# traceopt-ai/traceml

Hardware: AMD Instinct MI355X
Metric: instrumentation overhead (% step time) (lower is better)
Workload: dtype bf16; 1 GPU; model=resnet50, global_batch=256, image_size=224, parallelism=dp1, protocol=plain

## Files before the change

traceml_amd/models/resnet.py:

```python

from __future__ import annotations

import torch
import torch.nn as nn


class Bottleneck(nn.Module):
    expansion = 4

    def __init__(self, in_ch: int, width: int, stride: int = 1):
        super().__init__()
        out_ch = width * self.expansion
        self.conv1 = nn.Conv2d(in_ch, width, 1, bias=False)
        self.bn1 = nn.BatchNorm2d(width)
        self.conv2 = nn.Conv2d(width, width, 3, stride=stride, padding=1, bias=False)
        self.bn2 = nn.BatchNorm2d(width)
        self.conv3 = nn.Conv2d(width, out_ch, 1, bias=False)
        self.bn3 = nn.BatchNorm2d(out_ch)
        self.relu = nn.ReLU(inplace=True)
        self.downsample = None
        if stride != 1 or in_ch != out_ch:
            self.downsample = nn.Sequential(
                nn.Conv2d(in_ch, out_ch, 1, stride=stride, bias=False),
                nn.BatchNorm2d(out_ch),
            )

    def forward(self, x):
        identity = x
        out = self.relu(self.bn1(self.conv1(x)))
        out = self.relu(self.bn2(self.conv2(out)))
        out = self.bn3(self.conv3(out))
        if self.downsample is not None:
            identity = self.downsample(x)
        return self.relu(out + identity)


class ResNet(nn.Module):
    def __init__(self, layers, num_classes: int = 1000):
        super().__init__()
        self.in_ch = 64
        self.conv1 = nn.Conv2d(3, 64, 7, stride=2, padding=3, bias=False)
        self.bn1 = nn.BatchNorm2d(64)
        self.relu = nn.ReLU(inplace=True)
        self.maxpool = nn.MaxPool2d(3, stride=2, padding=1)
        self.layer1 = self._make_layer(64, layers[0], stride=1)
        self.layer2 = self._make_layer(128, layers[1], stride=2)
        self.layer3 = self._make_layer(256, layers[2], stride=2)
        self.layer4 = self._make_layer(512, layers[3], stride=2)
        self.avgpool = nn.AdaptiveAvgPool2d(1)
        self.fc = nn.Linear(512 * Bottleneck.expansion, num_classes)
        for m in self.modules():
            if isinstance(m, nn.Conv2d):
                nn.init.kaiming_normal_(m.weight, mode="fan_out", nonlinearity="relu")
            elif isinstance(m, nn.BatchNorm2d):
                nn.init.ones_(m.weight)
                nn.init.zeros_(m.bias)

    def _make_layer(self, width, blocks, stride):
        layers = [Bottleneck(self.in_ch, width, stride)]
        self.in_ch = width * Bottleneck.expansion
        layers += [Bottleneck(self.in_ch, width) for _ in range(blocks - 1)]
        return nn.Sequential(*layers)

    def forward(self, x):
        x = self.maxpool(self.relu(self.bn1(self.conv1(x))))
        x = self.layer4(self.layer3(self.layer2(self.layer1(x))))
        x = torch.flatten(self.avgpool(x), 1)
        return self.fc(x)


def resnet50(num_classes: int = 1000) -> ResNet:
    return ResNet([3, 4, 6, 3], num_classes=num_classes)
```

traceml_amd/ops/build_ext.py:

```python

from __future__ import annotations

import os
import subprocess
import sys
import sysconfig

HERE = os.path.dirname(os.path.abspath(__file__))
SRC = os.path.join(HERE, "hip", "traceml_hip.hip")


def extension_filename() -> str:
    suffix = sysconfig.get_config_var("EXT_SUFFIX") or ".so"
    return os.path.join(HERE, f"_traceml_hip{suffix}")


def _pybind11_include() -> str:
    import pybind11

    return pybind11.get_include()


def build(verbose: bool = True) -> str:
    out = extension_filename()
    python_include = sysconfig.get_paths()["include"]
    cmd = [
        "hipcc",
        "--offload-arch=gfx950",
        "-O3",
        "-std=c++17",
        "-fPIC",
        "-shared",
        f"-I{python_include}",
        f"-I{_pybind11_include()}",
        SRC,
        "-o",
        out,
    ]
    if verbose:
        print("+", " ".join(cmd), flush=True)
    env = dict(os.environ)
    env.setdefault("PYTORCH_ROCM_ARCH", "gfx950")
    subprocess.run(cmd, check=True, env=env)
    return out


def build_if_needed(verbose: bool = True) -> str:
    out = extension_filename()
    if os.path.exists(out) and os.path.getmtime(out) >= os.path.getmtime(SRC):
        return out
    return build(verbose=verbose)


if __name__ == "__main__":
    build()
```

traceml_amd/ops/hip/traceml_hip.hip:

```cpp

#include <hip/hip_runtime.h>
#include <pybind11/pybind11.h>

#include <atomic>
#include <chrono>
#include <cstdint>
#include <cstring>
#include <mutex>
#include <stdexcept>
#include <string>
#include <thread>
#include <vector>

namespace py = pybind11;

#define HIP_CHECK(expr)                                                        \
  do {                                                                         \
    hipError_t _err = (expr);                                                  \
    if (_err != hipSuccess) {                                                  \
      throw std::runtime_error(std::string("HIP error at " #expr ": ") +       \
                               hipGetErrorString(_err));                       \
    }                                                                          \
  } while (0)

struct Slot {
  unsigned long long ticks;
  unsigned long long seq;
};
static_assert(sizeof(Slot) == 16, "slot must be 16 bytes");


__global__ __launch_bounds__(64, 1) void stamp_kernel(Slot* __restrict__ ring,
                                                      unsigned long long mask,
                                                      unsigned long long seq) {
  __shared__ Slot staged;
  if (threadIdx.x == 0) {
    staged.ticks = __builtin_amdgcn_s_memrealtime();
    staged.seq = seq;
    Slot* slot = ring + (seq & mask);
    slot->ticks = staged.ticks;
    __hip_atomic_store(&slot->seq, staged.seq, __ATOMIC_RELEASE,
                       __HIP_MEMORY_SCOPE_SYSTEM);
  }
}


namespace {

struct RingState {
  Slot* host_ptr = nullptr;
  Slot* dev_ptr = nullptr;
  unsigned long long capacity = 0;
  unsigned long long mask = 0;
  std::atomic<unsigned long long> next_seq{1};
  double ticks_per_sec = 0.0;
  int device = -1;
  bool initialized = false;
};

RingState g_ring;
std::mutex g_init_mutex;

struct EventPool {
  std::vector<hipEvent_t> events;
  std::vector<int> free_ids;
  std::mutex mutex;
};

EventPool g_events;

unsigned long long round_up_pow2(unsigned long long v) {
  unsigned long long p = 1;
  while (p < v) p <<= 1;
  return p;
}

double query_wall_clock_rate(int device) {
  int khz = 0;
  hipError_t err =
      hipDeviceGetAttribute(&khz, hipDeviceAttributeWallClockRate, device);
  if (err != hipSuccess || khz <= 0) return 0.0;
  return static_cast<double>(khz) * 1000.0;
}

}


static unsigned long long ring_mark(uintptr_t stream_handle) {
  RingState& r = g_ring;
  unsigned long long seq = r.next_seq.fetch_add(1, std::memory_order_relaxed);
  hipStream_t stream = reinterpret_cast<hipStream_t>(stream_handle);
  stamp_kernel<<<1, 64, 0, stream>>>(r.dev_ptr, r.mask, seq);
  return seq;
}

static bool ring_ready(unsigned long long seq) {
  const RingState& r = g_ring;
  const Slot* slot = r.host_ptr + (seq & r.mask);
  unsigned long long observed = __atomic_load_n(&slot->seq, __ATOMIC_ACQUIRE);
  return observed == seq;
}

static long long ring_ticks(unsigned long long seq) {
  const RingState& r = g_ring;
  const Slot* slot = r.host_ptr + (seq & r.mask);
  unsigned long long observed = __atomic_load_n(&slot->seq, __ATOMIC_ACQUIRE);
  if (observed != seq) return -1;
  return static_cast<long long>(slot->ticks);
}

static double ring_elapsed_ms(unsigned long long seq_start,
                              unsigned long long seq_end) {
  long long t0 = ring_ticks(seq_start);
  long long t1 = ring_ticks(seq_end);
  if (t0 < 0 || t1 < 0) return -1.0;
  double dticks = static_cast<double>(t1 - t0);
  return dticks * 1000.0 / g_ring.ticks_per_sec;
}

static double calibrate(uintptr_t stream_handle, double window_sec) {
  hipStream_t stream = reinterpret_cast<hipStream_t>(stream_handle);
  unsigned long long a = ring_mark(reinterpret_cast<uintptr_t>(stream));
  HIP_CHECK(hipStreamSynchronize(stream));
  auto cpu0 = std::chrono::steady_clock::now();
  long long ta = ring_ticks(a);
  std::this_thread::sleep_for(
      std::chrono::microseconds(static_cast<long long>(window_sec * 1e6)));
  unsigned long long b = ring_mark(reinterpret_cast<uintptr_t>(stream));
  HIP_CHECK(hipStreamSynchronize(stream));
  auto cpu1 = std::chrono::steady_clock::now();
  long long tb = ring_ticks(b);
  double sec =
      std::chrono::duration_cast<std::chrono::duration<double>>(cpu1 - cpu0)
          .count();
  if (ta < 0 || tb < 0 || sec <= 0.0) {
    throw std::runtime_error("traceml_hip: calibration stamps did not land");
  }
  double rate = static_cast<double>(tb - ta) / sec;
  g_ring.ticks_per_sec = rate;
  return rate;
}

static void init(int device, unsigned long long slots) {
  std::lock_guard<std::mutex> guard(g_init_mutex);
  if (g_ring.initialized) return;
  HIP_CHECK(hipSetDevice(device));
  unsigned long long capacity = round_up_pow2(slots < 1024 ? 1024 : slots);
  void* host = nullptr;
  HIP_CHECK(hipHostMalloc(&host, capacity * sizeof(Slot),
                          hipHostMallocMapped | hipHostMallocCoherent));
  std::memset(host, 0, capacity * sizeof(Slot));
  void* dev = nullptr;
  HIP_CHECK(hipHostGetDevicePointer(&dev, host, 0));
  g_ring.host_ptr = static_cast<Slot*>(host);
  g_ring.dev_ptr = static_cast<Slot*>(dev);
  g_ring.capacity = capacity;
  g_ring.mask = capacity - 1;
  g_ring.device = device;
  g_ring.ticks_per_sec = query_wall_clock_rate(device);
  g_ring.initialized = true;
  try {
    calibrate(0, 0.050);
  } catch (const std::exception&) {
    if (g_ring.ticks_per_sec <= 0.0) g_ring.ticks_per_sec = 1.0e8;
  }
}

static bool is_initialized() { return g_ring.initialized; }

static double ticks_per_second() { return g_ring.ticks_per_sec; }


static int event_acquire() {
  std::lock_guard<std::mutex> guard(g_events.mutex);
  if (!g_events.free_ids.empty()) {
    int id = g_events.free_ids.back();
    g_events.free_ids.pop_back();
    return id;
  }
  hipEvent_t event;
  HIP_CHECK(hipEventCreateWithFlags(&event, hipEventDefault));
  g_events.events.push_back(event);
  return static_cast<int>(g_events.events.size()) - 1;
}

static hipEvent_t event_for(int id) {
  if (id < 0 || id >= static_cast<int>(g_events.events.size())) {
    throw std::runtime_error("traceml_hip: bad event id");
  }
  return g_events.events[static_cast<size_t>(id)];
}

static void event_record(int id, uintptr_t stream_handle) {
  HIP_CHECK(hipEventRecord(event_for(id),
                           reinterpret_cast<hipStream_t>(stream_handle)));
}

static bool event_query(int id) {
  hipError_t err = hipEventQuery(event_for(id));
  if (err == hipSuccess) return true;
  if (err == hipErrorNotReady) return false;
  HIP_CHECK(err);
  return false;
}

static double event_elapsed_ms(int start_id, int end_id) {
  float ms = 0.0f;
  HIP_CHECK(hipEventElapsedTime(&ms, event_for(start_id), event_for(end_id)));
  return static_cast<double>(ms);
}

static void event_release(int id) {
  std::lock_guard<std::mutex> guard(g_events.mutex);
  event_for(id);
  g_events.free_ids.push_back(id);
}

static int event_pool_size() {
  std::lock_guard<std::mutex> guard(g_events.mutex);
  return static_cast<int>(g_events.events.size());
}


PYBIND11_MODULE(_traceml_hip, m) {
  m.doc() = "traceml_amd MI355X-native timing: s_memrealtime ring stamps + "
            "hipEvent pool (gfx950)";
  m.def("init", &init, py::arg("device"), py::arg("slots") = 65536);
  m.def("is_initialized", &is_initialized);
  m.def("ticks_per_second", &ticks_per_second);
  m.def("ring_mark", &ring_mark, py::arg("stream"));
  m.def("ring_ready", &ring_ready, py::arg("seq"));
  m.def("ring_ticks", &ring_ticks, py::arg("seq"));
  m.def("ring_elapsed_ms", &ring_elapsed_ms, py::arg("seq_start"),
        py::arg("seq_end"));
  m.def("calibrate", &calibrate, py::arg("stream") = 0,
        py::arg("window_sec") = 0.05);
  m.def("event_acquire", &event_acquire);
  m.def("event_record", &event_record, py::arg("event_id"), py::arg("stream"));
  m.def("event_query", &event_query, py::arg("event_id"));
  m.def("event_elapsed_ms", &event_elapsed_ms, py::arg("start_id"),
        py::arg("end_id"));
  m.def("event_release", &event_release, py::arg("event_id"));
  m.def("event_pool_size", &event_pool_size);
}
```

Before: 0.1093 percent.

## Add fused BatchNorm+residual+ReLU HIP kernels for ResNet bottlenecks

Adds custom HIP kernels that fuse training-mode BatchNorm statistics, affine apply, residual add and ReLU for NHWC bf16 tensors, with matching backward kernels. ResNet blocks now route through bn_act, which falls back to the module path when hooks are present or shapes are unsupported. The aim is to cut memory traffic and kernel launches in the model step. This changes the step time that is the denominator of the overhead metric, and it also interacts with instrumentation, because hooked modules bypass the fused path.

```diff
diff --git a/profiles/fused_bn_bytes.py b/profiles/fused_bn_bytes.py
--- /dev/null
+++ b/profiles/fused_bn_bytes.py
@@ -0,0 +1,81 @@
+#!/usr/bin/env python3
+
+import csv
+import sys
+
+BATCH = 256
+ROOF_TBS = 6.29
+
+
+def plan_grid(rows, channels):
+    r = 256 // (channels // 8)
+    per_block = -(-rows // 1024)
+    per_block = -(-per_block // r) * r
+    per_block = max(per_block, 8 * r, 64)
+    return -(-rows // per_block)
+
+
+def sites():
+    out = [(BATCH * 112 * 112, 64, False)]
+    hw, in_planes = 56, 64
+    for width, blocks, stride in ((64, 3, 1), (128, 4, 2), (256, 6, 2),
+                                  (512, 3, 2)):
+        for b in range(blocks):
+            s = stride if b == 0 else 1
+            out.append((BATCH * hw * hw, width, False))
+            hw //= s
+            out.append((BATCH * hw * hw, width, False))
+            out.append((BATCH * hw * hw, width * 4, True))
+    return out
+
+
+def bytes_per_step():
+    total = {
+        "fbn_stats_partial": 0, "fbn_stats_finalize": 0,
+        "fbn_apply_forward": 0, "fbn_backward_reduce": 0,
+        "fbn_backward_finalize": 0, "fbn_backward_apply": 0,
+    }
+    for rows, c, res in sites():
+        t = rows * c * 2
+        part = plan_grid(rows, c) * 2 * c * 4
+        vec = c * 4
+        total["fbn_stats_partial"] += t + part
+        total["fbn_stats_finalize"] += part + 6 * vec
+        total["fbn_apply_forward"] += (3 if res else 2) * t + 4 * vec
+        total["fbn_backward_reduce"] += 3 * t + part + 2 * vec
+        total["fbn_backward_finalize"] += part + 2 * vec
+        total["fbn_backward_apply"] += (5 if res else 4) * t + 5 * vec
+    return total
+
+
+def main(argv):
+    per_step = bytes_per_step()
+    print(f"fused sites: {len(sites())}, elements per step: "
+          f"{sum(r * c for r, c, _ in sites()) / 1e9:.3f} G")
+    if len(argv) < 3:
+        for name, b in per_step.items():
+            print(f"{name:24s} {b / 1e9:8.3f} GB/step")
+        print(f"{'total':24s} {sum(per_step.values()) / 1e9:8.3f} GB/step")
+        return
+    steps = float(argv[2])
+    ns = dict.fromkeys(per_step, 0.0)
+    calls = dict.fromkeys(per_step, 0)
+    with open(argv[1], newline="") as fh:
+        for row in csv.DictReader(fh):
+            for name in per_step:
+                if name in row["Name"]:
+                    ns[name] += float(row["TotalDurationNs"])
+                    calls[name] += int(row["Calls"])
+    print("| kernel | launches/step | ms/step | GB/step | TB/s | of 6.29 TB/s |")
+    print("|---|---|---|---|---|---|")
+    for name, b in per_step.items():
+        ms = ns[name] / steps / 1e6
+        tbs = b / (ns[name] / steps) / 1e3 if ns[name] else 0.0
+        print(f"| `{name}` | {calls[name] / steps:.0f} | {ms:.3f} | "
+              f"{b / 1e9:.2f} | {tbs:.2f} | {100 * tbs / ROOF_TBS:.0f} % |")
+    print(f"| total | | {sum(ns.values()) / steps / 1e6:.3f} | "
+          f"{sum(per_step.values()) / 1e9:.2f} | | |")
+
+
+if __name__ == "__main__":
+    main(sys.argv)
diff --git a/traceml_amd/models/resnet.py b/traceml_amd/models/resnet.py
--- a/traceml_amd/models/resnet.py
+++ b/traceml_amd/models/resnet.py
@@ -3,6 +3,8 @@
 
 import torch
 import torch.nn as nn
+
+from traceml_amd.ops.fused_bn import bn_act
 
 
 class Bottleneck(nn.Module):
@@ -26,13 +28,14 @@
             )
 
     def forward(self, x):
-        identity = x
-        out = self.relu(self.bn1(self.conv1(x)))
-        out = self.relu(self.bn2(self.conv2(out)))
-        out = self.bn3(self.conv3(out))
-        if self.downsample is not None:
-            identity = self.downsample(x)
-        return self.relu(out + identity)
+        out = bn_act(self.conv1(x), self.bn1, relu=self.relu)
+        out = bn_act(self.conv2(out), self.bn2, relu=self.relu)
+        out = self.conv3(out)
+        if self.downsample is None:
+            return bn_act(out, self.bn3, residual=x, relu=self.relu)
+        return bn_act(
+            out, self.bn3, residual=lambda: self.downsample(x), relu=self.relu
+        )
 
 
 class ResNet(nn.Module):
@@ -63,7 +66,7 @@
         return nn.Sequential(*layers)
 
     def forward(self, x):
-        x = self.maxpool(self.relu(self.bn1(self.conv1(x))))
+        x = self.maxpool(bn_act(self.conv1(x), self.bn1, relu=self.relu))
         x = self.layer4(self.layer3(self.layer2(self.layer1(x))))
         x = torch.flatten(self.avgpool(x), 1)
         return self.fc(x)
diff --git a/traceml_amd/ops/build_ext.py b/traceml_amd/ops/build_ext.py
--- a/traceml_amd/ops/build_ext.py
+++ b/traceml_amd/ops/build_ext.py
@@ -8,6 +8,8 @@
 
 HERE = os.path.dirname(os.path.abspath(__file__))
 SRC = os.path.join(HERE, "hip", "traceml_hip.hip")
+SOURCES = [SRC, os.path.join(HERE, "hip", "fused_bn.hip")]
+HEADERS = [os.path.join(HERE, "hip", "fused_bn_plan.h")]
 
 
 def extension_filename() -> str:
@@ -33,7 +35,7 @@
         "-shared",
         f"-I{python_include}",
         f"-I{_pybind11_include()}",
-        SRC,
+        *SOURCES,
         "-o",
         out,
     ]
@@ -47,7 +49,9 @@
 
 def build_if_needed(verbose: bool = True) -> str:
     out = extension_filename()
-    if os.path.exists(out) and os.path.getmtime(out) >= os.path.getmtime(SRC):
+    if os.path.exists(out) and os.path.getmtime(out) >= max(
+        os.path.getmtime(f) for f in SOURCES + HEADERS
+    ):
         return out
     return build(verbose=verbose)
 
diff --git a/traceml_amd/ops/fused_bn.py b/traceml_amd/ops/fused_bn.py
--- /dev/null
+++ b/traceml_amd/ops/fused_bn.py
@@ -0,0 +1,247 @@
+
+from __future__ import annotations
+
+import os
+from typing import Callable, Optional, Union
+
+import torch
+import torch.nn as nn
+import torch.nn.functional as F
+from torch.autograd.function import once_differentiable
+from torch.nn.modules import module as _module_mod
+
+ENV_SWITCH = "TRACEML_FUSED_BN"
+
+_GLOBAL_HOOK_DICTS = (
+    "_global_forward_hooks",
+    "_global_forward_pre_hooks",
+    "_global_backward_hooks",
+    "_global_backward_pre_hooks",
+)
+_MODULE_HOOK_DICTS = (
+    "_forward_hooks",
+    "_forward_pre_hooks",
+    "_backward_hooks",
+    "_backward_pre_hooks",
+)
+
+
+def enabled() -> bool:
+    return os.environ.get(ENV_SWITCH, "1") != "0"
+
+
+def supported_channels(channels: int) -> bool:
+    if channels < 8 or channels > 2048 or channels % 8:
+        return False
+    return 256 % (channels // 8) == 0
+
+
+def _has_hooks(mod: Optional[nn.Module]) -> bool:
+    if mod is None:
+        return False
+    return any(getattr(mod, name, None) for name in _MODULE_HOOK_DICTS)
+
+
+def _global_hooks() -> bool:
+    return any(getattr(_module_mod, name, None) for name in _GLOBAL_HOOK_DICTS)
+
+
+def _dense_nhwc_bf16(t) -> bool:
+    return (
+        isinstance(t, torch.Tensor)
+        and t.is_cuda
+        and t.dtype == torch.bfloat16
+        and t.dim() == 4
+        and t.is_contiguous(memory_format=torch.channels_last)
+        and t.data_ptr() % 16 == 0
+    )
+
+
+def _fp32_vec(t, channels: int, device) -> bool:
+    return (
+        isinstance(t, torch.Tensor)
+        and t.dtype == torch.float32
+        and t.device == device
+        and t.dim() == 1
+        and t.numel() == channels
+        and t.is_contiguous()
+        and t.data_ptr() % 16 == 0
+    )
+
+
+def _module_ok(x, bn, relu_mod) -> bool:
+    if not enabled():
+        return False
+    if not _dense_nhwc_bf16(x):
+        return False
+    if type(bn) is not nn.BatchNorm2d:
+        return False
+    if not (bn.training and bn.track_running_stats and bn.affine):
+        return False
+    if bn.momentum is None or bn.weight is None or bn.bias is None:
+        return False
+    channels = x.shape[1]
+    if channels != bn.num_features or not supported_channels(channels):
+        return False
+    if x.numel() // channels < 2:
+        return False
+    if x.device.index != torch.cuda.current_device():
+        return False
+    for t in (bn.weight, bn.bias, bn.running_mean, bn.running_var):
+        if not _fp32_vec(t, channels, x.device):
+            return False
+    nbt = bn.num_batches_tracked
+    if not (
+        isinstance(nbt, torch.Tensor)
+        and nbt.dtype == torch.int64
+        and nbt.device == x.device
+        and nbt.numel() == 1
+    ):
+        return False
+    if _has_hooks(bn) or _has_hooks(relu_mod) or _global_hooks():
+        return False
+    return True
+
+
+def _residual_ok(x, residual) -> bool:
+    return (
+        _dense_nhwc_bf16(residual)
+        and residual.shape == x.shape
+        and residual.device == x.device
+    )
+
+
+def _extension():
+    from traceml_amd.ops import hip_ext
+
+    try:
+        return hip_ext.load_extension()
+    except ImportError as exc:
+        raise RuntimeError(
+            "fused BatchNorm needs the _traceml_hip extension; build it with "
+            "`python -m traceml_amd.ops.build_ext` (or set "
+            f"{ENV_SWITCH}=0 to use the module path)"
+        ) from exc
+
+
+def _workspace(ext, rows: int, channels: int, device):
+    return torch.empty(
+        ext.fused_bn_workspace_bytes(rows, channels),
+        dtype=torch.uint8,
+        device=device,
+    )
+
+
+class _FusedBNAct(torch.autograd.Function):
+
+    @staticmethod
+    def forward(ctx, x, residual, weight, bias, running_mean, running_var,
+                num_batches_tracked, eps, momentum, relu):
+        ext = _extension()
+        channels = x.shape[1]
+        rows = x.numel() // channels
+        y = torch.empty_like(x)
+        save_mean = torch.empty(channels, dtype=torch.float32, device=x.device)
+        save_invstd = torch.empty_like(save_mean)
+        ws = _workspace(ext, rows, channels, x.device)
+        ext.fused_bn_forward(
+            x.data_ptr(),
+            0 if residual is None else residual.data_ptr(),
+            y.data_ptr(),
+            weight.data_ptr(),
+            bias.data_ptr(),
+            running_mean.data_ptr(),
+            running_var.data_ptr(),
+            num_batches_tracked.data_ptr(),
+            save_mean.data_ptr(),
+            save_invstd.data_ptr(),
+            ws.data_ptr(),
+            ws.numel(),
+            rows,
+            channels,
+            float(eps),
+            float(momentum),
+            bool(relu),
+            torch.cuda.current_stream(x.device).cuda_stream,
+        )
+        ctx.save_for_backward(x, y, weight, save_mean, save_invstd)
+        ctx.relu = bool(relu)
+        ctx.has_residual = residual is not None
+        ctx.set_materialize_grads(False)
+        return y
+
+    @staticmethod
+    @once_differentiable
+    def backward(ctx, dy):
+        if dy is None:
+            return (None,) * 10
+        x, y, weight, save_mean, save_invstd = ctx.saved_tensors
+        ext = _extension()
+        channels = x.shape[1]
+        rows = x.numel() // channels
+        if dy.dtype != torch.bfloat16:
+            dy = dy.to(torch.bfloat16)
+        if not dy.is_contiguous(memory_format=torch.channels_last):
+            dy = dy.contiguous(memory_format=torch.channels_last)
+        if dy.data_ptr() % 16:
+            dy = dy.clone(memory_format=torch.channels_last)
+        dx = torch.empty_like(x)
+        d_res = torch.empty_like(x) if ctx.has_residual else None
+        grad_weight = torch.empty(channels, dtype=torch.float32, device=x.device)
+        grad_bias = torch.empty_like(grad_weight)
+        ws = _workspace(ext, rows, channels, x.device)
+        with torch.cuda.device(x.device):
+            ext.fused_bn_backward(
+                x.data_ptr(),
+                y.data_ptr() if ctx.relu else 0,
+                dy.data_ptr(),
+                weight.data_ptr(),
+                save_mean.data_ptr(),
+                save_invstd.data_ptr(),
+                dx.data_ptr(),
+                0 if d_res is None else d_res.data_ptr(),
+                grad_weight.data_ptr(),
+                grad_bias.data_ptr(),
+                ws.data_ptr(),
+                ws.numel(),
+                rows,
+                channels,
+                ctx.relu,
+                torch.cuda.current_stream(x.device).cuda_stream,
+            )
+        return (dx, d_res, grad_weight, grad_bias, None, None, None, None,
+                None, None)
+
+
+def fused_bn_act(x, residual, weight, bias, running_mean, running_var,
+                 num_batches_tracked, eps, momentum, relu):
+    return _FusedBNAct.apply(
+        x, residual, weight, bias, running_mean, running_var,
+        num_batches_tracked, eps, momentum, relu,
+    )
+
+
+def bn_act(
+    x: torch.Tensor,
+    bn: nn.BatchNorm2d,
+    residual: Union[None, torch.Tensor, Callable[[], torch.Tensor]] = None,
+    relu: Union[bool, nn.Module] = True,
+) -> torch.Tensor:
+    relu_mod = relu if isinstance(relu, nn.Module) else None
+    if _module_ok(x, bn, relu_mod):
+        res = residual() if callable(residual) else residual
+        if res is None or _residual_ok(x, res):
+            return fused_bn_act(
+                x, res, bn.weight, bn.bias, bn.running_mean, bn.running_var,
+                bn.num_batches_tracked, bn.eps, bn.momentum, bool(relu),
+            )
+        residual = res
+
+    out = bn(x)
+    if residual is not None:
+        out = out + (residual() if callable(residual) else residual)
+    if relu_mod is not None:
+        return relu_mod(out)
+    if relu:
+        return F.relu(out)
+    return out
diff --git a/traceml_amd/ops/hip/fused_bn.hip b/traceml_amd/ops/hip/fused_bn.hip
--- /dev/null
+++ b/traceml_amd/ops/hip/fused_bn.hip
@@ -0,0 +1,680 @@
+
+#include <hip/hip_runtime.h>
+#include <pybind11/pybind11.h>
+
+#include <cstdint>
+#include <stdexcept>
+#include <string>
+
+#include "fused_bn_plan.h"
+
+namespace py = pybind11;
+
+namespace {
+
+using fused_bn::kBlockThreads;
+using fused_bn::kFinalizeChannels;
+using fused_bn::kFinalizeLanes;
+
+#define FBN_HIP_CHECK(expr)                                                    \
+  do {                                                                         \
+    hipError_t _err = (expr);                                                  \
+    if (_err != hipSuccess) {                                                  \
+      throw std::runtime_error(std::string("HIP error at " #expr ": ") +       \
+                               hipGetErrorString(_err));                       \
+    }                                                                          \
+  } while (0)
+
+
+__device__ __forceinline__ void unpack8(const uint4& q, float (&f)[8]) {
+  f[0] = __uint_as_float(q.x << 16);
+  f[1] = __uint_as_float(q.x & 0xffff0000u);
+  f[2] = __uint_as_float(q.y << 16);
+  f[3] = __uint_as_float(q.y & 0xffff0000u);
+  f[4] = __uint_as_float(q.z << 16);
+  f[5] = __uint_as_float(q.z & 0xffff0000u);
+  f[6] = __uint_as_float(q.w << 16);
+  f[7] = __uint_as_float(q.w & 0xffff0000u);
+}
+
+__device__ __forceinline__ uint32_t bf16_bits(float f) {
+  uint32_t u = __float_as_uint(f);
+  if ((u & 0x7fffffffu) > 0x7f800000u) return 0x7fc0u;
+  u += 0x7fffu + ((u >> 16) & 1u);
+  return u >> 16;
+}
+
+__device__ __forceinline__ uint4 pack8(const float (&f)[8]) {
+  uint4 q;
+  q.x = bf16_bits(f[0]) | (bf16_bits(f[1]) << 16);
+  q.y = bf16_bits(f[2]) | (bf16_bits(f[3]) << 16);
+  q.z = bf16_bits(f[4]) | (bf16_bits(f[5]) << 16);
+  q.w = bf16_bits(f[6]) | (bf16_bits(f[7]) << 16);
+  return q;
+}
+
+__device__ __forceinline__ uint32_t mask_pair(uint32_t dy, uint32_t y) {
+  const uint32_t lo = y & 0xffffu;
+  const uint32_t hi = y >> 16;
+  const bool lo_pos = lo != 0u && lo <= 0x7f80u;
+  const bool hi_pos = hi != 0u && hi <= 0x7f80u;
+  return (lo_pos ? (dy & 0x0000ffffu) : 0u) | (hi_pos ? (dy & 0xffff0000u) : 0u);
+}
+
+__device__ __forceinline__ uint4 mask8(const uint4& dy, const uint4& y) {
+  uint4 q;
+  q.x = mask_pair(dy.x, y.x);
+  q.y = mask_pair(dy.y, y.y);
+  q.z = mask_pair(dy.z, y.z);
+  q.w = mask_pair(dy.w, y.w);
+  return q;
+}
+
+__device__ __forceinline__ void load8f(const float* p, float (&f)[8]) {
+  const float4 a = *reinterpret_cast<const float4*>(p);
+  const float4 b = *reinterpret_cast<const float4*>(p + 4);
+  f[0] = a.x; f[1] = a.y; f[2] = a.z; f[3] = a.w;
+  f[4] = b.x; f[5] = b.y; f[6] = b.z; f[7] = b.w;
+}
+
+__device__ __forceinline__ void store8f(float* p, const float (&f)[8]) {
+  *reinterpret_cast<float4*>(p) = make_float4(f[0], f[1], f[2], f[3]);
+  *reinterpret_cast<float4*>(p + 4) = make_float4(f[4], f[5], f[6], f[7]);
+}
+
+
+struct Geometry {
+  int vec;
+  int sub;
+  int rows_per_trip;
+  int64_t row_begin;
+  int64_t row_end;
+};
+
+__device__ __forceinline__ Geometry geometry(int64_t rows,
+                                             int64_t rows_per_block,
+                                             int vecs_per_row) {
+  Geometry g;
+  g.vec = fused_bn::thread_vec(static_cast<int>(threadIdx.x), vecs_per_row);
+  g.sub = fused_bn::thread_sub(static_cast<int>(threadIdx.x), vecs_per_row);
+  g.rows_per_trip = kBlockThreads / vecs_per_row;
+  g.row_begin = fused_bn::block_row_begin(blockIdx.x, rows_per_block, rows);
+  g.row_end = fused_bn::block_row_end(blockIdx.x, rows_per_block, rows);
+  return g;
+}
+
+
+struct Moments {
+  float n;
+  float mean[8];
+  float m2[8];
+};
+
+__device__ __forceinline__ void welford_row(Moments& s, const uint4& q) {
+  float x[8];
+  unpack8(q, x);
+  s.n += 1.0f;
+  const float inv_n = 1.0f / s.n;
+#pragma unroll
+  for (int j = 0; j < 8; ++j) {
+    const float d = x[j] - s.mean[j];
+    s.mean[j] = fmaf(d, inv_n, s.mean[j]);
+    s.m2[j] = fmaf(d, x[j] - s.mean[j], s.m2[j]);
+  }
+}
+
+__device__ __forceinline__ void chan_merge(float na, float& mean_a, float& m2_a,
+                                           float mean_b, float m2_b,
+                                           float frac_b) {
+  const float d = mean_b - mean_a;
+  mean_a = fmaf(d, frac_b, mean_a);
+  m2_a = m2_a + m2_b + d * d * (na * frac_b);
+}
+
+__global__ __launch_bounds__(kBlockThreads) void fbn_stats_partial_kernel(
+    const uint4* __restrict__ x, float* __restrict__ workspace, int64_t rows,
+    int64_t rows_per_block, int vecs_per_row) {
+  const Geometry g = geometry(rows, rows_per_block, vecs_per_row);
+  const int64_t V = vecs_per_row;
+  const int64_t R = g.rows_per_trip;
+  Moments s;
+  s.n = 0.0f;
+#pragma unroll
+  for (int j = 0; j < 8; ++j) {
+    s.mean[j] = 0.0f;
+    s.m2[j] = 0.0f;
+  }
+
+  int64_t r = g.row_begin + g.sub;
+  for (; r + 3 * R < g.row_end; r += 4 * R) {
+    const uint4 q0 = x[r * V + g.vec];
+    const uint4 q1 = x[(r + R) * V + g.vec];
+    const uint4 q2 = x[(r + 2 * R) * V + g.vec];
+    const uint4 q3 = x[(r + 3 * R) * V + g.vec];
+    welford_row(s, q0);
+    welford_row(s, q1);
+    welford_row(s, q2);
+    welford_row(s, q3);
+  }
+  for (; r < g.row_end; r += R) {
+    welford_row(s, x[r * V + g.vec]);
+  }
+
+  __shared__ float sh_mean[8 * kBlockThreads];
+  __shared__ float sh_m2[8 * kBlockThreads];
+  __shared__ float sh_n[kBlockThreads];
+  const int tid = static_cast<int>(threadIdx.x);
+  for (int half = g.rows_per_trip / 2; half >= 1; half >>= 1) {
+    if (g.sub >= half && g.sub < 2 * half) {
+      sh_n[tid] = s.n;
+#pragma unroll
+      for (int j = 0; j < 8; ++j) {
+        sh_mean[j * kBlockThreads + tid] = s.mean[j];
+        sh_m2[j * kBlockThreads + tid] = s.m2[j];
+      }
+    }
+    __syncthreads();
+    if (g.sub < half) {
+      const int other = tid + half * vecs_per_row;
+      const float nb = sh_n[other];
+      const float n = s.n + nb;
+      const float frac_b = n > 0.0f ? nb / n : 0.0f;
+#pragma unroll
+      for (int j = 0; j < 8; ++j) {
+        chan_merge(s.n, s.mean[j], s.m2[j],
+                   sh_mean[j * kBlockThreads + other],
+                   sh_m2[j * kBlockThreads + other], frac_b);
+      }
+      s.n = n;
+    }
+    __syncthreads();
+  }
+
+  if (g.sub == 0) {
+    const int64_t C = V * 8;
+    store8f(workspace + fused_bn::partial_offset(blockIdx.x, 0, C, g.vec * 8),
+            s.mean);
+    store8f(workspace + fused_bn::partial_offset(blockIdx.x, 1, C, g.vec * 8),
+            s.m2);
+  }
+}
+
+__global__ __launch_bounds__(kBlockThreads) void fbn_stats_finalize_kernel(
+    const float* __restrict__ workspace, int grid, int64_t rows,
+    int64_t rows_per_block, int channels, float eps, float momentum,
+    float* __restrict__ save_mean, float* __restrict__ save_invstd,
+    float* __restrict__ running_mean, float* __restrict__ running_var,
+    long long* __restrict__ num_batches_tracked) {
+  const int tid = static_cast<int>(threadIdx.x);
+  const int c = static_cast<int>(blockIdx.x) * kFinalizeChannels +
+                tid % kFinalizeChannels;
+  const int lane = tid / kFinalizeChannels;
+  const int64_t C = channels;
+
+  double n = 0.0, mean = 0.0, m2 = 0.0;
+  auto merge = [&](double nb, double mean_b, double m2_b) {
+    const double tot = n + nb;
+    if (tot > 0.0) {
+      const double d = mean_b - mean;
+      mean += d * (nb / tot);
+      m2 += m2_b + d * d * (n * nb / tot);
+    }
+    n = tot;
+  };
+  for (int p = lane; p < grid; p += kFinalizeLanes) {
+    const double nb = static_cast<double>(
+        fused_bn::block_row_end(p, rows_per_block, rows) -
+        fused_bn::block_row_begin(p, rows_per_block, rows));
+    merge(nb, workspace[fused_bn::partial_offset(p, 0, C, c)],
+          workspace[fused_bn::partial_offset(p, 1, C, c)]);
+  }
+
+  __shared__ double sh_n[kBlockThreads];
+  __shared__ double sh_mean[kBlockThreads];
+  __shared__ double sh_m2[kBlockThreads];
+  for (int half = kFinalizeLanes / 2; half >= 1; half >>= 1) {
+    if (lane >= half && lane < 2 * half) {
+      sh_n[tid] = n;
+      sh_mean[tid] = mean;
+      sh_m2[tid] = m2;
+    }
+    __syncthreads();
+    if (lane < half) {
+      const int other = tid + half * kFinalizeChannels;
+      merge(sh_n[other], sh_mean[other], sh_m2[other]);
+    }
+    __syncthreads();
+  }
+
+  if (lane == 0) {
+    const double count = static_cast<double>(rows);
+    const double var = m2 / count;
+    const double mom = static_cast<double>(momentum);
+    save_mean[c] = static_cast<float>(mean);
+    save_invstd[c] =
+        static_cast<float>(1.0 / sqrt(var + static_cast<double>(eps)));
+    const double unbiased = m2 / (count - 1.0);
+    running_mean[c] =
+        static_cast<float>((1.0 - mom) * running_mean[c] + mom * mean);
+    running_var[c] =
+        static_cast<float>((1.0 - mom) * running_var[c] + mom * unbiased);
+  }
+  if (blockIdx.x == 0 && tid == 0) {
+    *num_batches_tracked += 1;
+  }
+}
+
+
+template <bool kRelu, bool kResidual>
+__global__ __launch_bounds__(kBlockThreads) void fbn_apply_forward_kernel(
+    const uint4* __restrict__ x, const uint4* __restrict__ residual,
+    uint4* __restrict__ y, const float* __restrict__ weight,
+    const float* __restrict__ bias, const float* __restrict__ save_mean,
+    const float* __restrict__ save_invstd, int64_t rows,
+    int64_t rows_per_block, int vecs_per_row) {
+  const Geometry g = geometry(rows, rows_per_block, vecs_per_row);
+  const int64_t V = vecs_per_row;
+  const int64_t R = g.rows_per_trip;
+  float mean[8], scale[8], shift[8];
+  {
+    float w[8], istd[8];
+    load8f(weight + g.vec * 8, w);
+    load8f(save_invstd + g.vec * 8, istd);
+    load8f(save_mean + g.vec * 8, mean);
+    load8f(bias + g.vec * 8, shift);
+#pragma unroll
+    for (int j = 0; j < 8; ++j) scale[j] = w[j] * istd[j];
+  }
+
+  auto one = [&](const uint4& qx, const uint4& qr) {
+    float f[8], res[8];
+    unpack8(qx, f);
+    if (kResidual) unpack8(qr, res);
+#pragma unroll
+    for (int j = 0; j < 8; ++j) {
+      float v = fmaf(f[j] - mean[j], scale[j], shift[j]);
+      if (kResidual) v += res[j];
+      if (kRelu) v = v < 0.0f ? 0.0f : v;
+      f[j] = v;
+    }
+    return pack8(f);
+  };
+
+  int64_t r = g.row_begin + g.sub;
+  for (; r + 3 * R < g.row_end; r += 4 * R) {
+    const int64_t i0 = r * V + g.vec;
+    const int64_t i1 = (r + R) * V + g.vec;
+    const int64_t i2 = (r + 2 * R) * V + g.vec;
+    const int64_t i3 = (r + 3 * R) * V + g.vec;
+    const uint4 x0 = x[i0], x1 = x[i1], x2 = x[i2], x3 = x[i3];
+    uint4 r0 = x0, r1 = x1, r2 = x2, r3 = x3;
+    if (kResidual) {
+      r0 = residual[i0];
+      r1 = residual[i1];
+      r2 = residual[i2];
+      r3 = residual[i3];
+    }
+    y[i0] = one(x0, r0);
+    y[i1] = one(x1, r1);
+    y[i2] = one(x2, r2);
+    y[i3] = one(x3, r3);
+  }
+  for (; r < g.row_end; r += R) {
+    const int64_t i = r * V + g.vec;
+    const uint4 qx = x[i];
+    uint4 qr = qx;
+    if (kResidual) qr = residual[i];
+    y[i] = one(qx, qr);
+  }
+}
+
+
+template <bool kRelu>
+__global__ __launch_bounds__(kBlockThreads) void fbn_backward_reduce_kernel(
+    const uint4* __restrict__ x, const uint4* __restrict__ y,
+    const uint4* __restrict__ dy, const float* __restrict__ save_mean,
+    const float* __restrict__ save_invstd, float* __restrict__ workspace,
+    int64_t rows, int64_t rows_per_block, int vecs_per_row) {
+  const Geometry g = geometry(rows, rows_per_block, vecs_per_row);
+  const int64_t V = vecs_per_row;
+  const int64_t R = g.rows_per_trip;
+  float mean[8], istd[8], sum_dy[8], sum_dy_xhat[8];
+  load8f(save_mean + g.vec * 8, mean);
+  load8f(save_invstd + g.vec * 8, istd);
+#pragma unroll
+  for (int j = 0; j < 8; ++j) {
+    sum_dy[j] = 0.0f;
+    sum_dy_xhat[j] = 0.0f;
+  }
+
+  auto one = [&](const uint4& qx, const uint4& qy, const uint4& qdy) {
+    float fx[8], fg[8];
+    unpack8(qx, fx);
+    unpack8(kRelu ? mask8(qdy, qy) : qdy, fg);
+#pragma unroll
+    for (int j = 0; j < 8; ++j) {
+      const float xhat = (fx[j] - mean[j]) * istd[j];
+      sum_dy[j] += fg[j];
+      sum_dy_xhat[j] = fmaf(fg[j], xhat, sum_dy_xhat[j]);
+    }
+  };
+
+  int64_t r = g.row_begin + g.sub;
+  for (; r + R < g.row_end; r += 2 * R) {
+    const int64_t i0 = r * V + g.vec;
+    const int64_t i1 = (r + R) * V + g.vec;
+    const uint4 x0 = x[i0], x1 = x[i1];
+    const uint4 d0 = dy[i0], d1 = dy[i1];
+    uint4 y0 = d0, y1 = d1;
+    if (kRelu) {
+      y0 = y[i0];
+      y1 = y[i1];
+    }
+    one(x0, y0, d0);
+    one(x1, y1, d1);
+  }
+  for (; r < g.row_end; r += R) {
+    const int64_t i = r * V + g.vec;
+    const uint4 qx = x[i];
+    const uint4 qd = dy[i];
+    uint4 qy = qd;
+    if (kRelu) qy = y[i];
+    one(qx, qy, qd);
+  }
+
+  __shared__ float sh_a[8 * kBlockThreads];
+  __shared__ float sh_b[8 * kBlockThreads];
+  const int tid = static_cast<int>(threadIdx.x);
+  for (int half = g.rows_per_trip / 2; half >= 1; half >>= 1) {
+    if (g.sub >= half && g.sub < 2 * half) {
+#pragma unroll
+      for (int j = 0; j < 8; ++j) {
+        sh_a[j * kBlockThreads + tid] = sum_dy[j];
+        sh_b[j * kBlockThreads + tid] = sum_dy_xhat[j];
+      }
+    }
+    __syncthreads();
+    if (g.sub < half) {
+      const int other = tid + half * vecs_per_row;
+#pragma unroll
+      for (int j = 0; j < 8; ++j) {
+        sum_dy[j] += sh_a[j * kBlockThreads + other];
+        sum_dy_xhat[j] += sh_b[j * kBlockThreads + other];
+      }
+    }
+    __syncthreads();
+  }
+
+  if (g.sub == 0) {
+    const int64_t C = V * 8;
+    store8f(workspace + fused_bn::partial_offset(blockIdx.x, 0, C, g.vec * 8),
+            sum_dy);
+    store8f(workspace + fused_bn::partial_offset(blockIdx.x, 1, C, g.vec * 8),
+            sum_dy_xhat);
+  }
+}
+
+__global__ __launch_bounds__(kBlockThreads) void fbn_backward_finalize_kernel(
+    const float* __restrict__ workspace, int grid, int channels,
+    float* __restrict__ grad_weight, float* __restrict__ grad_bias) {
+  const int tid = static_cast<int>(threadIdx.x);
+  const int c = static_cast<int>(blockIdx.x) * kFinalizeChannels +
+                tid % kFinalizeChannels;
+  const int lane = tid / kFinalizeChannels;
+  const int64_t C = channels;
+
+  float a = 0.0f, b = 0.0f;
+  for (int p = lane; p < grid; p += kFinalizeLanes) {
+    a += workspace[fused_bn::partial_offset(p, 0, C, c)];
+    b += workspace[fused_bn::partial_offset(p, 1, C, c)];
+  }
+
+  __shared__ float sh_a[kBlockThreads];
+  __shared__ float sh_b[kBlockThreads];
+  for (int half = kFinalizeLanes / 2; half >= 1; half >>= 1) {
+    if (lane >= half && lane < 2 * half) {
+      sh_a[tid] = a;
+      sh_b[tid] = b;
+    }
+    __syncthreads();
+    if (lane < half) {
+      const int other = tid + half * kFinalizeChannels;
+      a += sh_a[other];
+      b += sh_b[other];
+    }
+    __syncthreads();
+  }
+  if (lane == 0) {
+    grad_bias[c] = a;
+    grad_weight[c] = b;
+  }
+}
+
+
+template <bool kRelu, bool kResidual>
+__global__ __launch_bounds__(kBlockThreads) void fbn_backward_apply_kernel(
+    const uint4* __restrict__ x, const uint4* __restrict__ y,
+    const uint4* __restrict__ dy, const float* __restrict__ weight,
+    const float* __restrict__ save_mean, const float* __restrict__ save_invstd,
+    const float* __restrict__ grad_weight, const float* __restrict__ grad_bias,
+    uint4* __restrict__ dx, uint4* __restrict__ d_residual, float inv_rows,
+    int64_t rows, int64_t rows_per_block, int vecs_per_row) {
+  const Geometry g = geometry(rows, rows_per_block, vecs_per_row);
+  const int64_t V = vecs_per_row;
+  const int64_t R = g.rows_per_trip;
+  float mean[8], istd[8], scale[8], c1[8], c2[8];
+  load8f(save_mean + g.vec * 8, mean);
+  load8f(save_invstd + g.vec * 8, istd);
+  load8f(weight + g.vec * 8, scale);
+  load8f(grad_bias + g.vec * 8, c1);
+  load8f(grad_weight + g.vec * 8, c2);
+#pragma unroll
+  for (int j = 0; j < 8; ++j) {
+    scale[j] *= istd[j];
+    c1[j] *= inv_rows;
+    c2[j] *= inv_rows;
+  }
+
+  auto one = [&](int64_t i, const uint4& qx, const uint4& qy, const uint4& qdy) {
+    const uint4 qg = kRelu ? mask8(qdy, qy) : qdy;
+    float fx[8], fg[8];
+    unpack8(qx, fx);
+    unpack8(qg, fg);
+#pragma unroll
+    for (int j = 0; j < 8; ++j) {
+      const float xhat = (fx[j] - mean[j]) * istd[j];
+      fx[j] = scale[j] * (fg[j] - c1[j] - xhat * c2[j]);
+    }
+    dx[i] = pack8(fx);
+    if (kResidual) d_residual[i] = qg;
+  };
+
+  int64_t r = g.row_begin + g.sub;
+  for (; r + R < g.row_end; r += 2 * R) {
+    const int64_t i0 = r * V + g.vec;
+    const int64_t i1 = (r + R) * V + g.vec;
+    const uint4 x0 = x[i0], x1 = x[i1];
+    const uint4 d0 = dy[i0], d1 = dy[i1];
+    uint4 y0 = d0, y1 = d1;
+    if (kRelu) {
+      y0 = y[i0];
+      y1 = y[i1];
+    }
+    one(i0, x0, y0, d0);
+    one(i1, x1, y1, d1);
+  }
+  for (; r < g.row_end; r += R) {
+    const int64_t i = r * V + g.vec;
+    const uint4 qx = x[i];
+    const uint4 qd = dy[i];
+    uint4 qy = qd;
+    if (kRelu) qy = y[i];
+    one(i, qx, qy, qd);
+  }
+}
+
+
+void require(bool ok, const char* what) {
+  if (!ok) throw std::invalid_argument(std::string("fused_bn: ") + what);
+}
+
+void require_ptr(uintptr_t p, const char* name) {
+  if (p == 0) {
+    throw std::invalid_argument(std::string("fused_bn: null pointer: ") + name);
+  }
+  if (p % 16 != 0) {
+    throw std::invalid_argument(
+        std::string("fused_bn: pointer not 16-byte aligned: ") + name);
+  }
+}
+
+fused_bn::Plan checked_plan(int64_t rows, int64_t channels, uintptr_t workspace,
+                            int64_t workspace_bytes) {
+  require(fused_bn::channels_supported(channels),
+          "unsupported channel count (need C % 8 == 0 and (C / 8) | 256)");
+  require(rows >= 2, "need at least 2 rows (M >= 2)");
+  fused_bn::Plan plan;
+  require(fused_bn::make_plan(rows, channels, &plan), "unsupported shape");
+  require_ptr(workspace, "workspace");
+  require(workspace_bytes >= plan.workspace_bytes, "workspace too small");
+  return plan;
+}
+
+int64_t workspace_bytes(int64_t rows, int64_t channels) {
+  fused_bn::Plan plan;
+  require(fused_bn::make_plan(rows, channels, &plan), "unsupported shape");
+  return plan.workspace_bytes;
+}
+
+template <typename T>
+T* as(uintptr_t p) {
+  return reinterpret_cast<T*>(p);
+}
+
+void forward(uintptr_t x, uintptr_t residual, uintptr_t y, uintptr_t weight,
+             uintptr_t bias, uintptr_t running_mean, uintptr_t running_var,
+             uintptr_t num_batches_tracked, uintptr_t save_mean,
+             uintptr_t save_invstd, uintptr_t workspace, int64_t ws_bytes,
+             int64_t rows, int64_t channels, double eps, double momentum,
+             bool relu, uintptr_t stream_handle) {
+  const fused_bn::Plan plan = checked_plan(rows, channels, workspace, ws_bytes);
+  require_ptr(x, "x");
+  require_ptr(y, "y");
+  if (residual != 0) require_ptr(residual, "residual");
+  require_ptr(weight, "weight");
+  require_ptr(bias, "bias");
+  require_ptr(running_mean, "running_mean");
+  require_ptr(running_var, "running_var");
+  require_ptr(save_mean, "save_mean");
+  require_ptr(save_invstd, "save_invstd");
+  require(num_batches_tracked != 0, "null pointer: num_batches_tracked");
+  require(num_batches_tracked % 8 == 0, "num_batches_tracked not 8-byte aligned");
+  require(eps > 0.0, "eps must be positive");
+
+  hipStream_t stream = reinterpret_cast<hipStream_t>(stream_handle);
+  const dim3 block(kBlockThreads);
+  fbn_stats_partial_kernel<<<dim3(plan.grid), block, 0, stream>>>(
+      as<const uint4>(x), as<float>(workspace), plan.rows, plan.rows_per_block,
+      plan.vecs_per_row);
+  fbn_stats_finalize_kernel<<<dim3(plan.finalize_grid), block, 0, stream>>>(
+      as<const float>(workspace), plan.grid, plan.rows, plan.rows_per_block,
+      plan.channels, static_cast<float>(eps), static_cast<float>(momentum),
+      as<float>(save_mean), as<float>(save_invstd), as<float>(running_mean),
+      as<float>(running_var), as<long long>(num_batches_tracked));
+#define FBN_APPLY(RELU, RES)                                                   \
+  fbn_apply_forward_kernel<RELU, RES><<<dim3(plan.grid), block, 0, stream>>>(  \
+      as<const uint4>(x), as<const uint4>(residual), as<uint4>(y),             \
+      as<const float>(weight), as<const float>(bias),                          \
+      as<const float>(save_mean), as<const float>(save_invstd), plan.rows,     \
+      plan.rows_per_block, plan.vecs_per_row)
+  if (relu) {
+    if (residual != 0) FBN_APPLY(true, true); else FBN_APPLY(true, false);
+  } else {
+    if (residual != 0) FBN_APPLY(false, true); else FBN_APPLY(false, false);
+  }
+#undef FBN_APPLY
+  FBN_HIP_CHECK(hipGetLastError());
+}
+
+void backward(uintptr_t x, uintptr_t y, uintptr_t dy, uintptr_t weight,
+              uintptr_t save_mean, uintptr_t save_invstd, uintptr_t dx,
+              uintptr_t d_residual, uintptr_t grad_weight, uintptr_t grad_bias,
+              uintptr_t workspace, int64_t ws_bytes, int64_t rows,
+              int64_t channels, bool relu, uintptr_t stream_handle) {
+  const fused_bn::Plan plan = checked_plan(rows, channels, workspace, ws_bytes);
+  require_ptr(x, "x");
+  if (relu) require_ptr(y, "y");
+  require_ptr(dy, "dy");
+  require_ptr(weight, "weight");
+  require_ptr(save_mean, "save_mean");
+  require_ptr(save_invstd, "save_invstd");
+  require_ptr(dx, "dx");
+  if (d_residual != 0) require_ptr(d_residual, "d_residual");
+  require_ptr(grad_weight, "grad_weight");
+  require_ptr(grad_bias, "grad_bias");
+
+  hipStream_t stream = reinterpret_cast<hipStream_t>(stream_handle);
+  const dim3 block(kBlockThreads);
+  const float inv_rows = static_cast<float>(1.0 / static_cast<double>(rows));
+#define FBN_REDUCE(RELU)                                                       \
+  fbn_backward_reduce_kernel<RELU><<<dim3(plan.grid), block, 0, stream>>>(     \
+      as<const uint4>(x), as<const uint4>(y), as<const uint4>(dy),             \
+      as<const float>(save_mean), as<const float>(save_invstd),                \
+      as<float>(workspace), plan.rows, plan.rows_per_block, plan.vecs_per_row)
+  if (relu) FBN_REDUCE(true); else FBN_REDUCE(false);
+#undef FBN_REDUCE
+  fbn_backward_finalize_kernel<<<dim3(plan.finalize_grid), block, 0, stream>>>(
+      as<const float>(workspace), plan.grid, plan.channels,
+      as<float>(grad_weight), as<float>(grad_bias));
+#define FBN_BWD(RELU, RES)                                                     \
+  fbn_backward_apply_kernel<RELU, RES><<<dim3(plan.grid), block, 0, stream>>>( \
+      as<const uint4>(x), as<const uint4>(y), as<const uint4>(dy),             \
+      as<const float>(weight), as<const float>(save_mean),                     \
+      as<const float>(save_invstd), as<const float>(grad_weight),              \
+      as<const float>(grad_bias), as<uint4>(dx), as<uint4>(d_residual),        \
+      inv_rows, plan.rows, plan.rows_per_block, plan.vecs_per_row)
+  if (relu) {
+    if (d_residual != 0) FBN_BWD(true, true); else FBN_BWD(true, false);
+  } else {
+    if (d_residual != 0) FBN_BWD(false, true); else FBN_BWD(false, false);
+  }
+#undef FBN_BWD
+  FBN_HIP_CHECK(hipGetLastError());
+}
+
+py::dict plan_dict(int64_t rows, int64_t channels) {
+  fused_bn::Plan plan;
+  require(fused_bn::make_plan(rows, channels, &plan), "unsupported shape");
+  py::dict d;
+  d["rows_per_trip"] = plan.rows_per_trip;
+  d["rows_per_block"] = plan.rows_per_block;
+  d["grid"] = plan.grid;
+  d["finalize_grid"] = plan.finalize_grid;
+  d["workspace_bytes"] = plan.workspace_bytes;
+  return d;
+}
+
+}
+
+void register_fused_bn(py::module_& m) {
+  m.def("fused_bn_supported_channels",
+        [](int64_t c) { return fused_bn::channels_supported(c); },
+        py::arg("channels"));
+  m.def("fused_bn_workspace_bytes", &workspace_bytes, py::arg("rows"),
+        py::arg("channels"));
+  m.def("fused_bn_plan", &plan_dict, py::arg("rows"), py::arg("channels"));
+  m.def("fused_bn_forward", &forward, py::arg("x"), py::arg("residual"),
+        py::arg("y"), py::arg("weight"), py::arg("bias"),
+        py::arg("running_mean"), py::arg("running_var"),
+        py::arg("num_batches_tracked"), py::arg("save_mean"),
+        py::arg("save_invstd"), py::arg("workspace"),
+        py::arg("workspace_bytes"), py::arg("rows"), py::arg("channels"),
+        py::arg("eps"), py::arg("momentum"), py::arg("relu"),
+        py::arg("stream"));
+  m.def("fused_bn_backward", &backward, py::arg("x"), py::arg("y"),
+        py::arg("dy"), py::arg("weight"), py::arg("save_mean"),
+        py::arg("save_invstd"), py::arg("dx"), py::arg("d_residual"),
+        py::arg("grad_weight"), py::arg("grad_bias"), py::arg("workspace"),
+        py::arg("workspace_bytes"), py::arg("rows"), py::arg("channels"),
+        py::arg("relu"), py::arg("stream"));
+}
diff --git a/traceml_amd/ops/hip/fused_bn_plan.h b/traceml_amd/ops/hip/fused_bn_plan.h
--- /dev/null
+++ b/traceml_amd/ops/hip/fused_bn_plan.h
@@ -0,0 +1,97 @@
+
+#pragma once
+
+#include <cstdint>
+
+#if defined(__HIPCC__)
+#define FUSED_BN_HD __host__ __device__
+#else
+#define FUSED_BN_HD
+#endif
+
+namespace fused_bn {
+
+constexpr int kBlockThreads = 256;
+constexpr int kVecElems = 8;
+constexpr int kMaxChannels = kBlockThreads * kVecElems;
+constexpr int64_t kTargetBlocks = 1024;
+constexpr int64_t kMinTrips = 8;
+constexpr int64_t kMinRows = 64;
+constexpr int kFinalizeChannels = 8;
+constexpr int kFinalizeLanes = kBlockThreads / kFinalizeChannels;
+
+struct Plan {
+  int64_t rows;
+  int channels;
+  int vecs_per_row;
+  int rows_per_trip;
+  int64_t rows_per_block;
+  int grid;
+  int finalize_grid;
+  int64_t workspace_bytes;
+};
+
+inline bool channels_supported(int64_t channels) {
+  if (channels < kVecElems || channels > kMaxChannels) return false;
+  if (channels % kVecElems != 0) return false;
+  return kBlockThreads % (channels / kVecElems) == 0;
+}
+
+constexpr int64_t kMaxRows = int64_t{1} << 40;
+
+inline bool make_plan(int64_t rows, int64_t channels, Plan* plan) {
+  if (!channels_supported(channels)) return false;
+  if (rows < 2 || rows > kMaxRows) return false;
+  Plan p;
+  p.rows = rows;
+  p.channels = static_cast<int>(channels);
+  p.vecs_per_row = p.channels / kVecElems;
+  p.rows_per_trip = kBlockThreads / p.vecs_per_row;
+  const int64_t r = p.rows_per_trip;
+  int64_t per_block = (rows + kTargetBlocks - 1) / kTargetBlocks;
+  per_block = (per_block + r - 1) / r * r;
+  const int64_t floor_rows = kMinTrips * r > kMinRows ? kMinTrips * r : kMinRows;
+  if (per_block < floor_rows) per_block = floor_rows;
+  p.rows_per_block = per_block;
+  p.grid = static_cast<int>((rows + per_block - 1) / per_block);
+  p.finalize_grid = p.channels / kFinalizeChannels;
+  p.workspace_bytes =
+      static_cast<int64_t>(p.grid) * 2 * p.channels *
+      static_cast<int64_t>(sizeof(float));
+  *plan = p;
+  return true;
+}
+
+
+FUSED_BN_HD inline int thread_vec(int thread, int vecs_per_row) {
+  return thread % vecs_per_row;
+}
+
+FUSED_BN_HD inline int thread_sub(int thread, int vecs_per_row) {
+  return thread / vecs_per_row;
+}
+
+FUSED_BN_HD inline int64_t block_row_begin(int64_t block,
+                                           int64_t rows_per_block,
+                                           int64_t rows) {
+  const int64_t b = block * rows_per_block;
+  return b < rows ? b : rows;
+}
+
+FUSED_BN_HD inline int64_t block_row_end(int64_t block, int64_t rows_per_block,
+                                         int64_t rows) {
+  const int64_t e = (block + 1) * rows_per_block;
+  return e < rows ? e : rows;
+}
+
+FUSED_BN_HD inline int64_t vector_index(int64_t row, int vecs_per_row,
+                                        int vec) {
+  return row * vecs_per_row + vec;
+}
+
+FUSED_BN_HD inline int64_t partial_offset(int64_t block, int which,
+                                          int64_t channels, int64_t channel) {
+  return (block * 2 + which) * channels + channel;
+}
+
+}
diff --git a/traceml_amd/ops/hip/traceml_hip.hip b/traceml_amd/ops/hip/traceml_hip.hip
--- a/traceml_amd/ops/hip/traceml_hip.hip
+++ b/traceml_amd/ops/hip/traceml_hip.hip
@@ -222,6 +222,8 @@
 }
 
 
+void register_fused_bn(py::module_& m);
+
 PYBIND11_MODULE(_traceml_hip, m) {
   m.doc() = "traceml_amd MI355X-native timing: s_memrealtime ring stamps + "
             "hipEvent pool (gfx950)";
@@ -242,4 +244,5 @@
         py::arg("end_id"));
   m.def("event_release", &event_release, py::arg("event_id"));
   m.def("event_pool_size", &event_pool_size);
-}
+  register_fused_bn(m);
+}
```

Result: slower. 0.2249 percent (+105.8%).
